# Hamedkiri/heuristique_style_transfer_code

Hardware: NVIDIA B200
Metric: images/sec (higher is better)
Workload: dtype tf32

## Files before the change

heuristique_style_transfer_code_b200/csrc/gramhead.cu:

```cuda
#include "../../include/gramhead.h"
#include "common.cuh"
#include "gram_fwd.cuh"
#include "gram_fwd_pair.cuh"
#include "gram_bwd.cuh"
#include "gram_bwd2.cuh"
#include "gram_bwd_pair.cuh"
#include "attn_head.cuh"
#include "umma_gemm.cuh"
#include "tgemm_pair.cuh"
#include "attn_head2.cuh"
#include "preprocess.cuh"
#include "transpose.cuh"
#include "patchgan.cuh"
#include "pool.cuh"
#include "stem.cuh"
#include "style_loss.cuh"
#include <string>

namespace gh {

static int sm_count_cached() {
  static int cached[64] = {0};
  int dev = 0;
  if (cudaGetDevice(&dev) != cudaSuccess || dev < 0 || dev >= 64) return 148;
// ... 309 lines not shown
          e3 = cudaFuncSetAttribute(gram_bwd_pair_kernel<KIND, MODE, NHWC, ATS, CH>,                                   \
                                    cudaFuncAttributeMaxDynamicSharedMemorySize, (int)kBpSmemBytes);                   \
          if (e3 != cudaSuccess) return (int)e3;                                                                       \
          gram_bwd_pair_kernel<KIND, MODE, NHWC, ATS, CH><<<2 * npairs, kBpThreads, kBpSmemBytes, st>>>(q, tmF, tmD);  \
        }
#define GH_LAUNCH_BP2(KIND, MODE, ATS, CH)                                                                             \
        {                                                                                                              \
          if (nhwc) GH_LAUNCH_BP(KIND, MODE, true, ATS, CH) else GH_LAUNCH_BP(KIND, MODE, false, ATS, CH)              \
        }
#define GH_LAUNCH_BP3(KIND)                                                                                            \
        {                                                                                                              \
          if (mode != GRAM_POOL) GH_LAUNCH_BP2(KIND, GRAM_DENSE, false, 1)                                             \
          else if (!ats) GH_LAUNCH_BP2(KIND, GRAM_POOL, false, 1)                                                      \
          else if (ch == 2) GH_LAUNCH_BP2(KIND, GRAM_POOL, true, 2)                                                    \
          else GH_LAUNCH_BP2(KIND, GRAM_POOL, true, 1)                                                                 \
        }
        if (is_bf16) GH_LAUNCH_BP3(KIND_BF16) else GH_LAUNCH_BP3(KIND_TF32)
#undef GH_LAUNCH_BP3
#undef GH_LAUNCH_BP2
#undef GH_LAUNCH_BP
        return (int)cudaGetLastError();
      }
    }
  }
  if (nhwc || df16) return GH_ERR_UNSUPPORTED;
  if (g_opt_bwd_variant == 2) {
    GramBwd2Params q;
    q.F = F; q.img_stride = img_stride; q.row_stride = row_stride;
    q.B = B; q.C = C; q.HW = HW; q.mode = mode;
    q.dP = dP; q.dp_img_stride = dp_img_stride; q.g = g; q.kshift = p.kshift; q.dG = dG;
    q.dF = dF; q.df_img_stride = df_img_stride; q.df_row_stride = df_row_stride; q.scale = p.scale;
    const int nhw = g_opt_bwd_nhw ? g_opt_bwd_nhw : 256;
    q.nHT = (HW + nhw - 1) / nhw;
    q.nCP = (C + 255) / 256;
    q.nkb = (C + 63) / 64;
    q.nA = (C > 128) ? 2 : 1;
    const long long total2 = (long long)B * q.nHT * q.nCP;
    if (total2 > 0x7fffffffLL) return GH_ERR_UNSUPPORTED;
    q.total_units = (int)total2;
    const int sms2 = sm_count_cached();
    const int ctas2 = (max_ctas > 0 && max_ctas < sms2) ? max_ctas : sms2;
    int grid2 = (int)(total2 < ctas2 ? total2 : ctas2);
    q.units_per_cta = (int)((total2 + grid2 - 1) / grid2);
    grid2 = (int)((total2 + q.units_per_cta - 1) / q.units_per_cta);
    q.df_vec_ok = (HW % 4 == 0 && df_img_stride % 4 == 0 && df_row_stride % 4 == 0 && ((uintptr_t)dF) % 16 == 0) ? 1 : 0;
    const bool s4 = (HW % 4 == 0) && (row_stride % 4 == 0) && (img_stride % 4 == 0);
    int src;
    if (f_dtype == GH_DTYPE_F32) src = (s4 && ((uintptr_t)F) % 16 == 0) ? 0 : 1;
    else src = (s4 && ((uintptr_t)F) % 8 == 0) ? 2 : 3;
    cudaError_t e2 = cudaErrorInvalidValue;
#define GH_LAUNCH_B2(SRC, NHW, NPW)                                                                                    \
    {                                                                                                                  \
      e2 = cudaFuncSetAttribute(gram_bwd2_kernel<SRC, NHW, NPW>, cudaFuncAttributeMaxDynamicSharedMemorySize,          \
                                (int)kB2SmemBytes);                                                                    \
      if (e2 == cudaSuccess) {                                                                                         \
        gram_bwd2_kernel<SRC, NHW, NPW><<<grid2, (NPW == 8 ? 13 : 20) * 32, kB2SmemBytes, st>>>(q);                    \
        e2 = cudaGetLastError();                                                                                       \
      }                                                                                                                \
    }
    if (nhw == 128) {
      if (src == 0) GH_LAUNCH_B2(0, 128, 8) else if (src == 1) GH_LAUNCH_B2(1, 128, 8)
      else if (src == 2) GH_LAUNCH_B2(2, 128, 8) else GH_LAUNCH_B2(3, 128, 8)
    } else if (g_opt_bwd_producer_warps == 8) {
      if (src == 0) GH_LAUNCH_B2(0, 256, 8) else if (src == 1) GH_LAUNCH_B2(1, 256, 8)
      else if (src == 2) GH_LAUNCH_B2(2, 256, 8) else GH_LAUNCH_B2(3, 256, 8)
    } else {
      if (src == 0) GH_LAUNCH_B2(0, 256, 16) else if (src == 1) GH_LAUNCH_B2(1, 256, 16)
      else if (src == 2) GH_LAUNCH_B2(2, 256, 16) else GH_LAUNCH_B2(3, 256, 16)
    }
#undef GH_LAUNCH_B2
    return (int)e2;
  }
  p.dF = dF; p.df_img_stride = df_img_stride; p.df_row_stride = df_row_stride;
  p.NB = (C > 256) ? 2 : 1;
  p.nHT = (HW + 127) / 128;
  p.nCB = (C + 256 * p.NB - 1) / (256 * p.NB);
  p.nkb = (C + 63) / 64;
  p.stage_bytes = kGbATileBytes + (uint32_t)p.NB * kGbBBlkBytes;
  p.stages = (int)(kGbRingBytes / p.stage_bytes);
  if (p.stages > kGbMaxStages) p.stages = kGbMaxStages;
  p.nacc = (p.NB == 1) ? 2 : 1;
  const long long total = (long long)B * p.nHT * p.nCB;
  if (total > 0x7fffffffLL) return GH_ERR_UNSUPPORTED;
  p.total_units = (int)total;
  const int sms = sm_count_cached();
  const int ctas = (max_ctas > 0 && max_ctas < sms) ? max_ctas : sms;
  const int grid = (int)(total < ctas ? total : ctas);
  cudaError_t e;
  if (f_dtype == GH_DTYPE_F32) {
    e = cudaFuncSetAttribute(gram_bwd_kernel<0>, cudaFuncAttributeMaxDynamicSharedMemorySize, (int)kGbSmemBytes);
    if (e != cudaSuccess) return (int)e;
    gram_bwd_kernel<0><<<grid, kGbThreads, kGbSmemBytes, st>>>(p);
  } else {
    e = cudaFuncSetAttribute(gram_bwd_kernel<2>, cudaFuncAttributeMaxDynamicSharedMemorySize, (int)kGbSmemBytes);
    if (e != cudaSuccess) return (int)e;
    gram_bwd_kernel<2><<<grid, kGbThreads, kGbSmemBytes, st>>>(p);
  }
  return (int)cudaGetLastError();
}

__device__ __forceinline__ int bin_start(int i, int C, int g) { return (int)(((long long)i * C) / g); }
__device__ __forceinline__ int bin_end(int i, int C, int g) { return (int)((((long long)(i + 1)) * C + g - 1) / g); }

__global__ void adaptive_pool_fwd_kernel(const float* __restrict__ G, int C, int g, float* __restrict__ desc,
                                         long long desc_img_stride) {
  const int i = blockIdx.x, b = blockIdx.y;
  const int r0 = bin_start(i, C, g), r1 = bin_end(i, C, g);
  const float* Gb = G + (long long)b * C * C;
  const int warp = threadIdx.x >> 5, lane = threadIdx.x & 31;
  for (int j = warp; j < g; j += 8) {
    const int c0 = bin_start(j, C, g), c1 = bin_end(j, C, g);
    const int w = c1 - c0, n = (r1 - r0) * w;
    float s = 0.f;
    for (int t = lane; t < n; t += 32) s += Gb[(long long)(r0 + t / w) * C + c0 + t % w];
#pragma unroll
    for (int o = 16; o > 0; o >>= 1) s += __shfl_xor_sync(0xffffffffu, s, o);
    if (lane == 0) desc[(long long)b * desc_img_stride + i * g + j] = s / (float)n;
  }
}
__global__ void adaptive_pool_bwd_kernel(const float* __restrict__ d_desc, long long desc_img_stride, int C, int g,
                                         float* __restrict__ dG) {
  const long long idx = (long long)blockIdx.x * blockDim.x + threadIdx.x;
  if (idx >= (long long)C * C) return;
  const int b = blockIdx.y;
  const int c = (int)(idx / C), d = (int)(idx % C);
  const float* dp = d_desc + (long long)b * desc_img_stride;
  int ilo = (int)(((long long)c * g) / C);
  while (ilo > 0 && bin_end(ilo - 1, C, g) > c) --ilo;
  int jlo = (int)(((long long)d * g) / C);
  while (jlo > 0 && bin_end(jlo - 1, C, g) > d) --jlo;
  float s = 0.f;
  for (int i = ilo; i < g && bin_start(i, C, g) <= c; ++i) {
    if (bin_end(i, C, g) <= c) continue;
    const float ni = (float)(bin_end(i, C, g) - bin_start(i, C, g));
    for (int j = jlo; j < g && bin_start(j, C, g) <= d; ++j) {
      if (bin_end(j, C, g) <= d) continue;
      const float nj = (float)(bin_end(j, C, g) - bin_start(j, C, g));
      s += dp[i * g + j] / (ni * nj);
    }
  }
  dG[(long long)b * C * C + idx] = s;
}

template <typename T>
static int stem_conv_pool_launch(StemConvPoolParams<T>& p, long long img_stride, long long c_stride, long long y_stride,
                                 long long x_stride, int B, int H, int W, void* stream) {
  p.s_img = img_stride; p.s_c = c_stride; p.s_y = y_stride; p.s_x = x_stride;
  p.B = B; p.OH = H / 2; p.OW = W / 2;
  p.PH = (p.OH - 1) / 2 + 1;
  p.PW = (p.OW - 1) / 2 + 1;
  p.tiles = (p.PW + kScTileCols - 1) / kScTileCols;
  p.vec2 = x_stride == 1 && (uintptr_t)p.x % (2 * sizeof(T)) == 0 && (img_stride % 2 == 0) && (c_stride % 2 == 0) &&
           (y_stride % 2 == 0);
  p.units = (long long)B * p.tiles * p.PH;
  const int sms = sm_count_cached();
  const int grid = (int)(p.units < sms ? p.units : sms);
  const uint32_t smem = sizeof(T) == 1 ? kScSmemBytesU8 : kScSmemBytes;
  cudaError_t e = cudaFuncSetAttribute(stem_conv_pool_kernel<T>, cudaFuncAttributeMaxDynamicSharedMemorySize, (int)smem);
  if (e != cudaSuccess) return (int)e;
  stem_conv_pool_kernel<T><<<grid, kScThreads, smem, (cudaStream_t)stream>>>(p);
  return (int)cudaGetLastError();
}

}

using namespace gh;

extern "C" {

int gh_version(void) { return 100; }

int gh_sm_count(void) { return sm_count_cached(); }

#ifdef GH_BP_PROFILE
int gh_bp_profile_read(unsigned long long* out) {
  unsigned long long zero[16] = {0};
  cudaError_t e = cudaDeviceSynchronize();
  if (e == cudaSuccess) e = cudaMemcpyFromSymbol(out, g_bp_prof, sizeof(zero));
  if (e == cudaSuccess) e = cudaMemcpyToSymbol(g_bp_prof, zero, sizeof(zero));
  return (int)e;
}
#endif

int gh_gram_bwd_plan(int C, int HW, int g, int f_dtype, int channels_last, int* out) {
  if (!out || C <= 0 || HW <= 0 || g <= 0 || (f_dtype != GH_DTYPE_F32 && f_dtype != GH_DTYPE_BF16)) return GH_ERR_BAD_ARG;
  if (C % g != 0 || g > kBpMaxG || C / g < 8 || ilog2_exact(C / g) < 0) return GH_ERR_UNSUPPORTED;
  GramBwdPairParams q;
  bool ats = false;
  int ch = 1;
  if (!plan_bwd_pair(C, HW, g, GRAM_POOL, f_dtype == GH_DTYPE_BF16, channels_last != 0, q, &ats, &ch)) return GH_ERR_UNSUPPORTED;
  out[0] = q.NT; out[1] = q.nHT; out[2] = ats ? 1 : 0; out[3] = ch; out[4] = q.a_stages; out[5] = q.b_stages;
  out[6] = q.a_tmem_base + q.a_stages * q.a_tmem_cols;
  out[7] = q.b_stages * q.b_stage_bytes + q.a_smem_tiles * (int)kBpTileBytes;
  return 0;
}

int gh_set_option(const char* name, int value) {
  if (!name) return GH_ERR_BAD_ARG;
  const std::string key(name);
  if (key == "gram_fwd_producer_warps") {
    if (value != 0 && value != 8 && value != 16) return GH_ERR_BAD_ARG;
    g_opt_fwd_producer_warps = value;
    return 0;
  }
  if (key == "gram_fwd_pair") {
    if (value < -1 || value > 1) return GH_ERR_BAD_ARG;
    g_opt_fwd_pair = value;
    return 0;
  }
  if (key == "gram_bwd_pair") {
    if (value < -1 || value > 1) return GH_ERR_BAD_ARG;
    g_opt_bwd_pair = value;
    return 0;
  }
  if (key == "gram_bwd_nt") {
    if (value != 0 && (value < 64 || value > 256 || value % 16)) return GH_ERR_BAD_ARG;
    g_opt_bwd_nt = value;
    return 0;
  }
  if (key == "gram_bwd_stages") {
    const int a = value >> 4, b = value & 15;
    if (value != 0 && (a < kBpGroups || b < 2 || a > kBpRingTiles - 2 || b > kBpMaxStages)) return GH_ERR_BAD_ARG;
    g_opt_bwd_stages = value;
    return 0;
  }
  if (key == "gram_bwd_ats") {
    if (value < -1 || value > 1) return GH_ERR_BAD_ARG;
    g_opt_bwd_ats = value;
    return 0;
  }
  if (key == "gram_bwd_ch") {
    if (value < 0 || value > 2) return GH_ERR_BAD_ARG;
    g_opt_bwd_ch = value;
    return 0;
  }
  if (key == "tma_f32_type") {
    if (value != 0 && value != 1) return GH_ERR_BAD_ARG;
    g_opt_tma_f32_type = value;
    return 0;
  }
  if (key == "gram_fwd_epilogue_warps") {
    if (value != 0 && value != 4 && value != 8) return GH_ERR_BAD_ARG;
    g_opt_fwd_epilogue_warps = value;
    return 0;
  }
  if (key == "tgemm_tn") {
    if (value != 0 && value != 128 && value != 256) return GH_ERR_BAD_ARG;
    g_opt_tg_tn = value;
    return 0;
  }
  if (key == "pdl") {
    if (value != 0 && value != 1) return GH_ERR_BAD_ARG;
    g_opt_pdl = value;
    return 0;
  }
  if (key == "attn_gemm") {
    if (value != 0 && value != 1) return GH_ERR_BAD_ARG;
    g_opt_attn_gemm = value;
    return 0;
  }
  if (key == "gram_bwd_variant") {
    if (value != 1 && value != 2) return GH_ERR_BAD_ARG;
    g_opt_bwd_variant = value;
    return 0;
  }
  if (key == "gram_bwd_producer_warps") {
    if (value != 8 && value != 16) return GH_ERR_BAD_ARG;
    g_opt_bwd_producer_warps = value;
    return 0;
  }
  if (key == "gram_bwd_nhw") {
    if (value != 0 && value != 128 && value != 256) return GH_ERR_BAD_ARG;
    g_opt_bwd_nhw = value;
    return 0;
  }
  return GH_ERR_BAD_ARG;
}

int gh_last_device_error(unsigned int* out4) {
  if (!out4) return GH_ERR_BAD_ARG;
  volatile unsigned int* rec = error_record_host();
  if (!rec) return GH_ERR_UNSUPPORTED;
  for (int i = 0; i < 4; ++i) out4[i] = rec[i];
  for (int i = 3; i >= 0; --i) rec[i] = 0u;
  return 0;
}

int gh_gram_pool_fwd(const void* F, int f_dtype, long long img_stride, long long row_stride, long long x_stride, int B,
                     int C, int HW, int g, float* desc, int l, int L, int ksplit, int max_ctas, void* stream) {
  if (!desc || l < 0 || l >= L || g <= 0) return GH_ERR_BAD_ARG;
  return gram_fwd_common(F, f_dtype, img_stride, row_stride, x_stride, B, C, HW, GRAM_POOL, g, desc + (long long)l * g * g,
                         (long long)L * g * g, ksplit, max_ctas, (cudaStream_t)stream);
}

int gh_gram_dense_fwd(const void* F, int f_dtype, long long img_stride, long long row_stride, long long x_stride, int B,
                      int C, int HW, float* G, int ksplit, int max_ctas, void* stream) {
  return gram_fwd_common(F, f_dtype, img_stride, row_stride, x_stride, B, C, HW, GRAM_DENSE, 0, G, (long long)C * C, ksplit,
                         max_ctas, (cudaStream_t)stream);
}

int gh_adaptive_pool_fwd(const float* G, int B, int C, int g, float* desc, int l, int L, void* stream) {
  if (!G || !desc || B <= 0 || C <= 0 || g <= 0 || l < 0 || l >= L) return GH_ERR_BAD_ARG;
  if (B > 65535) return GH_ERR_UNSUPPORTED;
  adaptive_pool_fwd_kernel<<<dim3(g, B), 256, 0, (cudaStream_t)stream>>>(G, C, g, desc + (long long)l * g * g,
                                                                         (long long)L * g * g);
  return (int)cudaGetLastError();
}

int gh_adaptive_pool_bwd(const float* d_desc, int l, int L, int B, int C, int g, float* dG, void* stream) {
  if (!dG || !d_desc || B <= 0 || C <= 0 || g <= 0 || l < 0 || l >= L) return GH_ERR_BAD_ARG;
  if (B > 65535) return GH_ERR_UNSUPPORTED;
  const long long n = (long long)C * C;
  adaptive_pool_bwd_kernel<<<dim3((unsigned)((n + 255) / 256), B), 256, 0, (cudaStream_t)stream>>>(
      d_desc + (long long)l * g * g, (long long)L * g * g, C, g, dG);
  return (int)cudaGetLastError();
}

int gh_gram_pool_bwd(const void* F, int f_dtype, long long img_stride, long long row_stride, long long x_stride, int B,
                     int C, int HW, int g, const float* d_desc, int l, int L, void* dF, int df_dtype,
                     long long df_img_stride, long long df_row_stride, long long df_x_stride, int max_ctas, void* stream) {
  if (!d_desc || l < 0 || l >= L || g <= 0) return GH_ERR_BAD_ARG;
  return gram_bwd_common(F, f_dtype, img_stride, row_stride, x_stride, B, C, HW, GRAM_POOL, g,
                         d_desc + (long long)l * g * g, (long long)L * g * g, nullptr, dF, df_dtype, df_img_stride,
                         df_row_stride, df_x_stride, max_ctas, (cudaStream_t)stream);
}

int gh_gram_dense_bwd(const void* F, int f_dtype, long long img_stride, long long row_stride, long long x_stride, int B,
                      int C, int HW, const float* dG, void* dF, int df_dtype, long long df_img_stride,
                      long long df_row_stride, long long df_x_stride, int max_ctas, void* stream) {
  return gram_bwd_common(F, f_dtype, img_stride, row_stride, x_stride, B, C, HW, GRAM_DENSE, 0, nullptr, 0, dG, dF,
                         df_dtype, df_img_stride, df_row_stride, df_x_stride, max_ctas, (cudaStream_t)stream);
}
// ... 443 lines not shown
```

heuristique_style_transfer_code_b200/csrc/stem.cuh:

```cuda
#pragma once
#include "common.cuh"
#include "preprocess.cuh"

namespace gh {

constexpr int kScProducerWarps = 8;
constexpr int kScEpiWarp0 = 8;
constexpr int kScMmaWarp = 12;
constexpr int kScThreads = 13 * 32;
constexpr int kScTileCols = 63;
constexpr int kScCells = 131;
constexpr int kScItems = 3 * kScCells;
constexpr int kScItemIters = (kScItems + 31) / 32;
constexpr int kScSlots = 12;
constexpr int kScAccSlots = 8;
constexpr uint32_t kScSlotBytes = kScCells * 16;
constexpr uint32_t kScPlaneBytes = kScSlots * kScSlotBytes;
constexpr uint32_t kScWBytes = 16 * 2 * 2048;
constexpr uint32_t kScAOff = kScWBytes;
constexpr uint32_t kScBiasOff = kScAOff + 4 * kScPlaneBytes;
constexpr uint32_t kScXbufOff = kScBiasOff + 64 * 4;
constexpr uint32_t kScBarOff = kScXbufOff + 2 * 4 * 64 * 4;
constexpr uint32_t kScBarBytes = 8 * (2 * kScSlots + 2 * kScAccSlots) + 16;
constexpr uint32_t kScSmemBytes = kScBarOff + kScBarBytes + 1024;
constexpr uint32_t kScTableOff = kScBarOff + kScBarBytes;
constexpr uint32_t kScSmemBytesU8 = kScSmemBytes + 3 * 256 * 4;

template <typename T>
struct StemConvPoolParams {
  const T* x;
  long long s_img, s_c, s_y, s_x;
  const float* w;
  const float* bias;
  float* out;
  int B, OH, OW, PH, PW, tiles;
  int vec2;
  long long units;
  float mean[3], std[3];
};

__device__ __forceinline__ float max_nan(float a, float b) { return (b > a || b != b) ? b : a; }

struct ScSeg {
  int b, j, py0, py1, y_lo, y_hi;
};
template <typename T>
__device__ __forceinline__ bool sc_next(const StemConvPoolParams<T>& p, long long& u, long long u1, ScSeg& s) {
  if (u >= u1) return false;
  const long long bj = u / p.PH;
  const long long end = (bj + 1) * p.PH < u1 ? (bj + 1) * p.PH : u1;
  s.b = (int)(bj / p.tiles);
  s.j = (int)(bj - (long long)s.b * p.tiles);
  s.py0 = (int)(u - bj * p.PH);
  s.py1 = s.py0 + (int)(end - u);
  s.y_lo = 2 * s.py0 - 1 > 0 ? 2 * s.py0 - 1 : 0;
  s.y_hi = 2 * s.py1 - 1 < p.OH - 1 ? 2 * s.py1 - 1 : p.OH - 1;
  u = end;
  return true;
}

__device__ __forceinline__ float4 sc_load_block(const StemConvPoolParams<float>& p, const float* q, const float*) {
  if (p.vec2) {
    const float2 t0 = __ldg(reinterpret_cast<const float2*>(q));
    const float2 t1 = __ldg(reinterpret_cast<const float2*>(q + p.s_y));
    return make_float4(t0.x, t0.y, t1.x, t1.y);
  }
  return make_float4(__ldg(q), __ldg(q + p.s_x), __ldg(q + p.s_y), __ldg(q + p.s_y + p.s_x));
}

__device__ __forceinline__ float4 sc_load_block(const StemConvPoolParams<uint8_t>& p, const uint8_t* q,
                                                const float* table) {
  uint32_t b0, b1, b2, b3;
  if (p.vec2) {
    const uint32_t t0 = __ldg(reinterpret_cast<const unsigned short*>(q));
    const uint32_t t1 = __ldg(reinterpret_cast<const unsigned short*>(q + p.s_y));
    b0 = t0 & 0xffu; b1 = t0 >> 8; b2 = t1 & 0xffu; b3 = t1 >> 8;
  } else {
    b0 = __ldg(q); b1 = __ldg(q + p.s_x); b2 = __ldg(q + p.s_y); b3 = __ldg(q + p.s_y + p.s_x);
  }
  return make_float4(table[b0], table[b1], table[b2], table[b3]);
}

template <typename T>
__global__ void __launch_bounds__(kScThreads, 1) stem_conv_pool_kernel(const StemConvPoolParams<T> p) {
  extern __shared__ uint8_t smem_raw[];
  const uint32_t raw = smem_u32(smem_raw);
  const uint32_t base = (raw + 1023u) & ~1023u;
  uint8_t* gbase = smem_raw + (base - raw);
  const uint32_t w_smem = base, a_smem = base + kScAOff;
  const float* bias_s = reinterpret_cast<const float*>(gbase + kScBiasOff);
  float* xbuf = reinterpret_cast<float*>(gbase + kScXbufOff);
  const uint32_t bar_full = base + kScBarOff, bar_empty = bar_full + 8 * kScSlots;
  const uint32_t bar_afull = bar_empty + 8 * kScSlots, bar_aempty = bar_afull + 8 * kScAccSlots;
  const uint32_t tmem_slot = bar_aempty + 8 * kScAccSlots;
  volatile uint32_t* tmem_slot_ptr = reinterpret_cast<volatile uint32_t*>(gbase + (tmem_slot - base));
  const int warp = threadIdx.x >> 5, lane = threadIdx.x & 31;

  {
    const float4* wg = reinterpret_cast<const float4*>(p.w);
    float4* ws = reinterpret_cast<float4*>(gbase);
    for (int i = threadIdx.x; i < (int)(kScWBytes / 16); i += kScThreads) ws[i] = __ldg(wg + i);
    if (threadIdx.x < 64) reinterpret_cast<float*>(gbase + kScBiasOff)[threadIdx.x] = __ldg(p.bias + threadIdx.x);
    float4* z = reinterpret_cast<float4*>(gbase + kScAOff + 3 * kScPlaneBytes);
    for (int i = threadIdx.x; i < (int)(kScPlaneBytes / 16); i += kScThreads) z[i] = make_float4(0.f, 0.f, 0.f, 0.f);
    if constexpr (sizeof(T) == 1) {
      float* table = reinterpret_cast<float*>(gbase + kScTableOff);
      for (int i = threadIdx.x; i < 3 * 256; i += kScThreads) {
        const int c = i >> 8;
        table[i] = to_tensor_normalize((unsigned)(i & 255), c == 0 ? p.mean[0] : c == 1 ? p.mean[1] : p.mean[2],
                                       c == 0 ? p.std[0] : c == 1 ? p.std[1] : p.std[2]);
      }
    }
    fence_proxy_async_smem();
  }
  if (threadIdx.x == 0) {
    for (int s = 0; s < kScSlots; ++s) {
      mbar_init(bar_full + 8 * s, 1);
      mbar_init(bar_empty + 8 * s, 1);
    }
    for (int s = 0; s < kScAccSlots; ++s) {
      mbar_init(bar_afull + 8 * s, 1);
      mbar_init(bar_aempty + 8 * s, 4);
    }
    mbar_fence_init();
  }
  if (warp == kScMmaWarp) tmem_alloc(tmem_slot, 512);
  tc_fence_before_sync();
  __syncthreads();
  tc_fence_after_sync();
  const uint32_t tmem_base = *tmem_slot_ptr;

  const long long u0 = p.units * blockIdx.x / gridDim.x, u1 = p.units * (blockIdx.x + 1) / gridDim.x;

  if (warp < kScProducerWarps) {
    uint32_t gs = 0;
    long long u = u0;
    ScSeg sg;
    while (sc_next(p, u, u1, sg)) {
      const int n_stage = sg.y_hi - sg.y_lo + 4;
      const T* img = p.x + (long long)sg.b * p.s_img;
      for (int k = 0; k < n_stage; ++k) {
        const uint32_t g = gs + (uint32_t)k;
        if ((int)(g % kScProducerWarps) != warp) continue;
        const uint32_t slot = g % kScSlots;
        const int Y = sg.y_lo + k - 2;
        const bool row_ok = Y >= 0 && Y < p.OH;
        float4 v[kScItemIters];
#pragma unroll
        for (int it = 0; it < kScItemIters; ++it) {
          const int i = it * 32 + lane;
          const int c = i / kScCells, s = i - c * kScCells;
          const int X = kScTileCols * 2 * sg.j + s - 3;
          v[it] = make_float4(0.f, 0.f, 0.f, 0.f);
          if (i < kScItems && row_ok && X >= 0 && X < p.OW) {
            const T* q = img + (long long)c * p.s_c + (long long)(2 * Y) * p.s_y + (long long)(2 * X) * p.s_x;
            v[it] = sc_load_block(p, q, reinterpret_cast<const float*>(gbase + kScTableOff) + c * 256);
          }
        }
        mbar_wait(bar_empty + 8 * slot, ((g / kScSlots) & 1u) ^ 1u, 300u + slot);
#pragma unroll
        for (int it = 0; it < kScItemIters; ++it) {
          const int i = it * 32 + lane;
          if (i < kScItems) {
            const int c = i / kScCells, s = i - c * kScCells;
            sts_u4(a_smem + (uint32_t)c * kScPlaneBytes + slot * kScSlotBytes + (uint32_t)s * 16u, tf32_rna(v[it].x),
                   tf32_rna(v[it].y), tf32_rna(v[it].z), tf32_rna(v[it].w));
          }
        }
        fence_proxy_async_smem();
        __syncwarp();
        if (lane == 0) mbar_arrive(bar_full + 8 * slot);
      }
      gs += (uint32_t)n_stage;
    }
  } else if (warp == kScMmaWarp) {
    constexpr uint32_t idesc = make_idesc_tf32(128, 64);
    const uint64_t adesc0 = make_smem_desc_noswz(a_smem, kScPlaneBytes, 128);
    const uint64_t bdesc0 = make_smem_desc_noswz(w_smem, 1024, 128);
    uint32_t gs = 0, gc = 0;
    long long u = u0;
    ScSeg sg;
    while (sc_next(p, u, u1, sg)) {
      const int n_conv = sg.y_hi - sg.y_lo + 1;
      for (int k = 0; k < n_conv; ++k, ++gc) {
        const uint32_t acc = gc % kScAccSlots;
        mbar_wait(bar_aempty + 8 * acc, ((gc / kScAccSlots) & 1u) ^ 1u, 400u + acc);
        uint32_t slot[4];
#pragma unroll
        for (int a = 0; a < 4; ++a) {
          const uint32_t g = gs + (uint32_t)(k + a);
          slot[a] = g % kScSlots;
          mbar_wait(bar_full + 8 * slot[a], (g / kScSlots) & 1u, 500u + slot[a]);
        }
        tc_fence_after_sync();
        if (elect_one()) {
          const uint32_t d = tmem_base + acc * 64u;
#pragma unroll
          for (int a = 0; a < 4; ++a) {
            const uint64_t arow = adesc0 + ((slot[a] * kScSlotBytes) >> 4);
#pragma unroll
            for (int b = 0; b < 4; ++b)
#pragma unroll
              for (int h = 0; h < 2; ++h) {
                const uint64_t da = arow + ((b * 16 + h * 2 * kScPlaneBytes) >> 4);
                const uint64_t db = bdesc0 + ((((a * 4 + b) * 2 + h) * 2048) >> 4);
                umma_tf32(d, da, db, idesc, (a | b | h) != 0);
              }
          }
          umma_commit(bar_afull + 8 * acc);
          umma_commit(bar_empty + 8 * slot[0]);
          if (k == n_conv - 1)
            for (int a = 1; a < 4; ++a) umma_commit(bar_empty + 8 * slot[a]);
        }
        __syncwarp();
      }
      gs += (uint32_t)(n_conv + 3);
    }
  } else {
    const int quad = warp - kScEpiWarp0;
    const uint32_t tlane = tmem_base + ((uint32_t)(32 * quad) << 16);
    const float neg_inf = -__int_as_float(0x7f800000);
    uint32_t gc = 0, xb = 0;
    long long u = u0;
    ScSeg sg;
    while (sc_next(p, u, u1, sg)) {
      const int x = kScTileCols * 2 * sg.j - 1 + 32 * quad + lane;
      const bool col_ok = x >= 0 && x < p.OW;
      auto acc_of = [&](int y) { return (gc + (uint32_t)(y - sg.y_lo)) % kScAccSlots; };
      auto wait_row = [&](int y) {
        const uint32_t g = gc + (uint32_t)(y - sg.y_lo);
        mbar_wait(bar_afull + 8 * (g % kScAccSlots), (g / kScAccSlots) & 1u, 600u + g % kScAccSlots);
      };
      for (int py = sg.py0; py < sg.py1; ++py) {
        const int ya = 2 * py - 1, yb = 2 * py, yc = 2 * py + 1;
        const bool ha = ya >= sg.y_lo, hc = yc <= sg.y_hi;
        if (py == sg.py0 && ha) wait_row(ya);
        wait_row(yb);
        if (hc) wait_row(yc);
        tc_fence_after_sync();
        float m[64];
#pragma unroll
        for (int h = 0; h < 2; ++h) {
          uint32_t r[32];
          tmem_ld32_nowait(tlane + acc_of(yb) * 64u + 32u * h, r);
          tmem_ld_wait();
#pragma unroll
          for (int i = 0; i < 32; ++i) m[32 * h + i] = __uint_as_float(r[i]);
          if (ha) {
            tmem_ld32_nowait(tlane + acc_of(ya) * 64u + 32u * h, r);
            tmem_ld_wait();
#pragma unroll
            for (int i = 0; i < 32; ++i) m[32 * h + i] = max_nan(m[32 * h + i], __uint_as_float(r[i]));
          }
          if (hc) {
            tmem_ld32_nowait(tlane + acc_of(yc) * 64u + 32u * h, r);
            tmem_ld_wait();
#pragma unroll
            for (int i = 0; i < 32; ++i) m[32 * h + i] = max_nan(m[32 * h + i], __uint_as_float(r[i]));
          }
        }
        tc_fence_before_sync();
        __syncwarp();
        if (lane == 0) {
          if (ha) mbar_arrive(bar_aempty + 8 * acc_of(ya));
          mbar_arrive(bar_aempty + 8 * acc_of(yb));
          if (hc && py == sg.py1 - 1) mbar_arrive(bar_aempty + 8 * acc_of(yc));
        }
        if (!col_ok) {
#pragma unroll
          for (int i = 0; i < 64; ++i) m[i] = neg_inf;
        }
        float* xs = xbuf + xb * 256;
        if (lane == 0 && quad > 0) {
#pragma unroll
          for (int i = 0; i < 64; i += 4)
            *reinterpret_cast<float4*>(xs + quad * 64 + i) = make_float4(m[i], m[i + 1], m[i + 2], m[i + 3]);
        }
        asm volatile("bar.sync 1, 128;" ::: "memory");
        const bool from_next = lane == 30 && quad < 3;
        const int qx = 16 * quad + (lane >> 1);
        const int px = kScTileCols * sg.j + qx;
        const bool store = !(lane & 1) && qx < kScTileCols && px < p.PW;
        float4* o = reinterpret_cast<float4*>(p.out + (((long long)sg.b * p.PH + py) * p.PW + px) * 64);
#pragma unroll
        for (int i = 0; i < 64; i += 4) {
          float r4[4];
#pragma unroll
          for (int e = 0; e < 4; ++e) {
            const float v1 = __shfl_down_sync(0xffffffffu, m[i + e], 1);
            float v2 = __shfl_down_sync(0xffffffffu, m[i + e], 2);
            if (from_next) v2 = xs[(quad + 1) * 64 + i + e];
            float t = max_nan(max_nan(m[i + e], v1), v2) + bias_s[i + e];
            r4[e] = t != t ? t : fmaxf(t, 0.f);
          }
          if (store) o[i / 4] = make_float4(r4[0], r4[1], r4[2], r4[3]);
        }
        xb ^= 1u;
      }
      gc += (uint32_t)(sg.y_hi - sg.y_lo + 1);
    }
  }

  tc_fence_before_sync();
  __syncthreads();
  if (warp == kScMmaWarp) {
    tc_fence_after_sync();
    tmem_dealloc(tmem_base, 512);
  }
}

}
```

Before: 43890.

## Rebalance stem conv-pool warps, split epilogue by channel halves, trim UMMA work

Reassigns warps in the stem conv+pool kernel: seven producer warps and eight epilogue warps, with each group of four epilogue warps handling one half of the 64 output channels and using its own named barrier. The epilogue now issues its TMEM loads back to back and carries the bottom conv row forward in registers, so each accumulator row is loaded once instead of twice. The MMA issue skips the zero third plane for odd k-steps by using separate descriptors, which removes the zero-filled plane and its shared memory. It also swaps the hand-written NaN-propagating max for the max.NaN instruction, moves unit indexing to 32-bit, and adds optional clock64 profiling. The risks are lower producer throughput with one fewer warp and correctness of the new descriptor strides.

After: 45960, median of 6. 1.05x the previous value.

```diff
diff --git a/heuristique_style_transfer_code_b200/csrc/gramhead.cu b/heuristique_style_transfer_code_b200/csrc/gramhead.cu
--- a/heuristique_style_transfer_code_b200/csrc/gramhead.cu
+++ b/heuristique_style_transfer_code_b200/csrc/gramhead.cu
@@ -485,9 +485,11 @@
   p.tiles = (p.PW + kScTileCols - 1) / kScTileCols;
   p.vec2 = x_stride == 1 && (uintptr_t)p.x % (2 * sizeof(T)) == 0 && (img_stride % 2 == 0) && (c_stride % 2 == 0) &&
            (y_stride % 2 == 0);
-  p.units = (long long)B * p.tiles * p.PH;
+  const long long units = (long long)B * p.tiles * p.PH;
+  if (units >= (1ll << 30)) return GH_ERR_UNSUPPORTED;
+  p.units = (int)units;
   const int sms = sm_count_cached();
-  const int grid = (int)(p.units < sms ? p.units : sms);
+  const int grid = p.units < sms ? p.units : sms;
   const uint32_t smem = sizeof(T) == 1 ? kScSmemBytesU8 : kScSmemBytes;
   cudaError_t e = cudaFuncSetAttribute(stem_conv_pool_kernel<T>, cudaFuncAttributeMaxDynamicSharedMemorySize, (int)smem);
   if (e != cudaSuccess) return (int)e;
@@ -511,6 +513,16 @@
   cudaError_t e = cudaDeviceSynchronize();
   if (e == cudaSuccess) e = cudaMemcpyFromSymbol(out, g_bp_prof, sizeof(zero));
   if (e == cudaSuccess) e = cudaMemcpyToSymbol(g_bp_prof, zero, sizeof(zero));
+  return (int)e;
+}
+#endif
+
+#ifdef GH_SC_PROFILE
+int gh_sc_profile_read(unsigned long long* out) {
+  unsigned long long zero[16] = {0};
+  cudaError_t e = cudaDeviceSynchronize();
+  if (e == cudaSuccess) e = cudaMemcpyFromSymbol(out, g_sc_prof, sizeof(zero));
+  if (e == cudaSuccess) e = cudaMemcpyToSymbol(g_sc_prof, zero, sizeof(zero));
   return (int)e;
 }
 #endif
diff --git a/heuristique_style_transfer_code_b200/csrc/stem.cuh b/heuristique_style_transfer_code_b200/csrc/stem.cuh
--- a/heuristique_style_transfer_code_b200/csrc/stem.cuh
+++ b/heuristique_style_transfer_code_b200/csrc/stem.cuh
@@ -4,10 +4,11 @@
 
 namespace gh {
 
-constexpr int kScProducerWarps = 8;
-constexpr int kScEpiWarp0 = 8;
-constexpr int kScMmaWarp = 12;
-constexpr int kScThreads = 13 * 32;
+constexpr int kScProducerWarps = 7;
+constexpr int kScEpiWarp0 = kScProducerWarps;
+constexpr int kScEpiWarps = 8;
+constexpr int kScMmaWarp = kScEpiWarp0 + kScEpiWarps;
+constexpr int kScThreads = (kScMmaWarp + 1) * 32;
 constexpr int kScTileCols = 63;
 constexpr int kScCells = 131;
 constexpr int kScItems = 3 * kScCells;
@@ -18,7 +19,7 @@
 constexpr uint32_t kScPlaneBytes = kScSlots * kScSlotBytes;
 constexpr uint32_t kScWBytes = 16 * 2 * 2048;
 constexpr uint32_t kScAOff = kScWBytes;
-constexpr uint32_t kScBiasOff = kScAOff + 4 * kScPlaneBytes;
+constexpr uint32_t kScBiasOff = kScAOff + 3 * kScPlaneBytes;
 constexpr uint32_t kScXbufOff = kScBiasOff + 64 * 4;
 constexpr uint32_t kScBarOff = kScXbufOff + 2 * 4 * 64 * 4;
 constexpr uint32_t kScBarBytes = 8 * (2 * kScSlots + 2 * kScAccSlots) + 16;
@@ -35,24 +36,43 @@
   float* out;
   int B, OH, OW, PH, PW, tiles;
   int vec2;
-  long long units;
+  int units;
   float mean[3], std[3];
 };
 
-__device__ __forceinline__ float max_nan(float a, float b) { return (b > a || b != b) ? b : a; }
+#ifdef GH_SC_PROFILE
+__device__ unsigned long long g_sc_prof[16];
+#define GH_SC_DECL(var) long long var = 0
+#define GH_SC_CLK(var) const long long var = clock64()
+#define GH_SC_ADD(acc, var) acc += clock64() - var
+#define GH_SC_FLUSH(slot, acc) atomicAdd(&g_sc_prof[slot], (unsigned long long)(acc))
+#define GH_SC_INC(var) ++var
+#else
+#define GH_SC_DECL(var)
+#define GH_SC_CLK(var)
+#define GH_SC_ADD(acc, var)
+#define GH_SC_FLUSH(slot, acc)
+#define GH_SC_INC(var)
+#endif
+
+__device__ __forceinline__ float max_nan(float a, float b) {
+  float r;
+  asm("max.NaN.f32 %0, %1, %2;" : "=f"(r) : "f"(a), "f"(b));
+  return r;
+}
 
 struct ScSeg {
   int b, j, py0, py1, y_lo, y_hi;
 };
 template <typename T>
-__device__ __forceinline__ bool sc_next(const StemConvPoolParams<T>& p, long long& u, long long u1, ScSeg& s) {
+__device__ __forceinline__ bool sc_next(const StemConvPoolParams<T>& p, int& u, int u1, ScSeg& s) {
   if (u >= u1) return false;
-  const long long bj = u / p.PH;
-  const long long end = (bj + 1) * p.PH < u1 ? (bj + 1) * p.PH : u1;
-  s.b = (int)(bj / p.tiles);
-  s.j = (int)(bj - (long long)s.b * p.tiles);
-  s.py0 = (int)(u - bj * p.PH);
-  s.py1 = s.py0 + (int)(end - u);
+  const int bj = u / p.PH;
+  const int end = (bj + 1) * p.PH < u1 ? (bj + 1) * p.PH : u1;
+  s.b = bj / p.tiles;
+  s.j = bj - s.b * p.tiles;
+  s.py0 = u - bj * p.PH;
+  s.py1 = s.py0 + (end - u);
   s.y_lo = 2 * s.py0 - 1 > 0 ? 2 * s.py0 - 1 : 0;
   s.y_hi = 2 * s.py1 - 1 < p.OH - 1 ? 2 * s.py1 - 1 : p.OH - 1;
   u = end;
@@ -83,6 +103,7 @@
 
 template <typename T>
 __global__ void __launch_bounds__(kScThreads, 1) stem_conv_pool_kernel(const StemConvPoolParams<T> p) {
+  GH_SC_CLK(prof_cta0);
   extern __shared__ uint8_t smem_raw[];
   const uint32_t raw = smem_u32(smem_raw);
   const uint32_t base = (raw + 1023u) & ~1023u;
@@ -101,8 +122,6 @@
     float4* ws = reinterpret_cast<float4*>(gbase);
     for (int i = threadIdx.x; i < (int)(kScWBytes / 16); i += kScThreads) ws[i] = __ldg(wg + i);
     if (threadIdx.x < 64) reinterpret_cast<float*>(gbase + kScBiasOff)[threadIdx.x] = __ldg(p.bias + threadIdx.x);
-    float4* z = reinterpret_cast<float4*>(gbase + kScAOff + 3 * kScPlaneBytes);
-    for (int i = threadIdx.x; i < (int)(kScPlaneBytes / 16); i += kScThreads) z[i] = make_float4(0.f, 0.f, 0.f, 0.f);
     if constexpr (sizeof(T) == 1) {
       float* table = reinterpret_cast<float*>(gbase + kScTableOff);
       for (int i = threadIdx.x; i < 3 * 256; i += kScThreads) {
@@ -120,7 +139,7 @@
     }
     for (int s = 0; s < kScAccSlots; ++s) {
       mbar_init(bar_afull + 8 * s, 1);
-      mbar_init(bar_aempty + 8 * s, 4);
+      mbar_init(bar_aempty + 8 * s, kScEpiWarps);
     }
     mbar_fence_init();
   }
@@ -130,12 +149,17 @@
   tc_fence_after_sync();
   const uint32_t tmem_base = *tmem_slot_ptr;
 
-  const long long u0 = p.units * blockIdx.x / gridDim.x, u1 = p.units * (blockIdx.x + 1) / gridDim.x;
+  const int u0 = (int)((long long)p.units * blockIdx.x / gridDim.x);
+  const int u1 = (int)((long long)p.units * (blockIdx.x + 1) / gridDim.x);
 
   if (warp < kScProducerWarps) {
     uint32_t gs = 0;
-    long long u = u0;
+    int u = u0;
     ScSeg sg;
+    GH_SC_DECL(prof_wait);
+    GH_SC_DECL(prof_store);
+    GH_SC_DECL(prof_n);
+    GH_SC_CLK(prof_t0);
     while (sc_next(p, u, u1, sg)) {
       const int n_stage = sg.y_hi - sg.y_lo + 4;
       const T* img = p.x + (long long)sg.b * p.s_img;
@@ -157,7 +181,11 @@
             v[it] = sc_load_block(p, q, reinterpret_cast<const float*>(gbase + kScTableOff) + c * 256);
           }
         }
+        GH_SC_CLK(prof_w0);
         mbar_wait(bar_empty + 8 * slot, ((g / kScSlots) & 1u) ^ 1u, 300u + slot);
+        GH_SC_ADD(prof_wait, prof_w0);
+        GH_SC_CLK(prof_s0);
+        GH_SC_INC(prof_n);
 #pragma unroll
         for (int it = 0; it < kScItemIters; ++it) {
           const int i = it * 32 + lane;
@@ -170,21 +198,40 @@
         fence_proxy_async_smem();
         __syncwarp();
         if (lane == 0) mbar_arrive(bar_full + 8 * slot);
+        GH_SC_ADD(prof_store, prof_s0);
       }
       gs += (uint32_t)n_stage;
     }
+#ifdef GH_SC_PROFILE
+    if (warp == 0 && lane == 0) {
+      long long prof_tot = 0;
+      GH_SC_ADD(prof_tot, prof_t0);
+      GH_SC_FLUSH(4, prof_tot);
+      GH_SC_FLUSH(5, prof_wait);
+      GH_SC_FLUSH(6, prof_store);
+      GH_SC_FLUSH(7, prof_n);
+    }
+#endif
   } else if (warp == kScMmaWarp) {
     constexpr uint32_t idesc = make_idesc_tf32(128, 64);
     const uint64_t adesc0 = make_smem_desc_noswz(a_smem, kScPlaneBytes, 128);
     const uint64_t bdesc0 = make_smem_desc_noswz(w_smem, 1024, 128);
+    const uint64_t adesc2 = make_smem_desc_noswz(a_smem + 2 * kScPlaneBytes, 16, 128);
+    const uint64_t bdesc2 = make_smem_desc_noswz(w_smem + 2048, 4096, 128);
     uint32_t gs = 0, gc = 0;
-    long long u = u0;
+    int u = u0;
     ScSeg sg;
+    GH_SC_DECL(prof_ae);
+    GH_SC_DECL(prof_full);
+    GH_SC_CLK(prof_t0);
     while (sc_next(p, u, u1, sg)) {
       const int n_conv = sg.y_hi - sg.y_lo + 1;
       for (int k = 0; k < n_conv; ++k, ++gc) {
         const uint32_t acc = gc % kScAccSlots;
+        GH_SC_CLK(prof_w0);
         mbar_wait(bar_aempty + 8 * acc, ((gc / kScAccSlots) & 1u) ^ 1u, 400u + acc);
+        GH_SC_ADD(prof_ae, prof_w0);
+        GH_SC_CLK(prof_w1);
         uint32_t slot[4];
 #pragma unroll
         for (int a = 0; a < 4; ++a) {
@@ -192,20 +239,19 @@
           slot[a] = g % kScSlots;
           mbar_wait(bar_full + 8 * slot[a], (g / kScSlots) & 1u, 500u + slot[a]);
         }
+        GH_SC_ADD(prof_full, prof_w1);
         tc_fence_after_sync();
         if (elect_one()) {
           const uint32_t d = tmem_base + acc * 64u;
 #pragma unroll
           for (int a = 0; a < 4; ++a) {
-            const uint64_t arow = adesc0 + ((slot[a] * kScSlotBytes) >> 4);
+            const uint32_t row = (slot[a] * kScSlotBytes) >> 4;
 #pragma unroll
             for (int b = 0; b < 4; ++b)
-#pragma unroll
-              for (int h = 0; h < 2; ++h) {
-                const uint64_t da = arow + ((b * 16 + h * 2 * kScPlaneBytes) >> 4);
-                const uint64_t db = bdesc0 + ((((a * 4 + b) * 2 + h) * 2048) >> 4);
-                umma_tf32(d, da, db, idesc, (a | b | h) != 0);
-              }
+              umma_tf32(d, adesc0 + row + b, bdesc0 + (((a * 4 + b) * 2 * 2048) >> 4), idesc, (a | b) != 0);
+#pragma unroll
+            for (int b = 0; b < 4; b += 2)
+              umma_tf32(d, adesc2 + row + b, bdesc2 + (((a * 4 + b) * 2 * 2048) >> 4), idesc, 1u);
           }
           umma_commit(bar_afull + 8 * acc);
           umma_commit(bar_empty + 8 * slot[0]);
@@ -216,13 +262,30 @@
       }
       gs += (uint32_t)(n_conv + 3);
     }
+#ifdef GH_SC_PROFILE
+    if (lane == 0) {
+      long long prof_tot = 0;
+      GH_SC_ADD(prof_tot, prof_t0);
+      GH_SC_FLUSH(0, prof_tot);
+      GH_SC_FLUSH(1, prof_ae);
+      GH_SC_FLUSH(2, prof_full);
+      GH_SC_FLUSH(3, gc);
+    }
+#endif
   } else {
-    const int quad = warp - kScEpiWarp0;
-    const uint32_t tlane = tmem_base + ((uint32_t)(32 * quad) << 16);
+    const int quad = warp & 3, half = (warp - kScEpiWarp0) >> 2;
+    const uint32_t tlane = tmem_base + ((uint32_t)(32 * quad) << 16) + 32u * (uint32_t)half;
+    const float* bias_h = bias_s + 32 * half;
     const float neg_inf = -__int_as_float(0x7f800000);
     uint32_t gc = 0, xb = 0;
-    long long u = u0;
+    int u = u0;
     ScSeg sg;
+    GH_SC_DECL(prof_af);
+    GH_SC_DECL(prof_ld);
+    GH_SC_DECL(prof_bar);
+    GH_SC_DECL(prof_st);
+    GH_SC_DECL(prof_n);
+    GH_SC_CLK(prof_t0);
     while (sc_next(p, u, u1, sg)) {
       const int x = kScTileCols * 2 * sg.j - 1 + 32 * quad + lane;
       const bool col_ok = x >= 0 && x < p.OW;
@@ -231,74 +294,88 @@
         const uint32_t g = gc + (uint32_t)(y - sg.y_lo);
         mbar_wait(bar_afull + 8 * (g % kScAccSlots), (g / kScAccSlots) & 1u, 600u + g % kScAccSlots);
       };
+      uint32_t ra[32];
       for (int py = sg.py0; py < sg.py1; ++py) {
         const int ya = 2 * py - 1, yb = 2 * py, yc = 2 * py + 1;
-        const bool ha = ya >= sg.y_lo, hc = yc <= sg.y_hi;
-        if (py == sg.py0 && ha) wait_row(ya);
+        const bool ha = ya >= sg.y_lo, hc = yc <= sg.y_hi, first = py == sg.py0;
+        GH_SC_CLK(prof_w0);
+        if (first && ha) wait_row(ya);
         wait_row(yb);
         if (hc) wait_row(yc);
+        GH_SC_ADD(prof_af, prof_w0);
+        GH_SC_CLK(prof_l0);
+        GH_SC_INC(prof_n);
         tc_fence_after_sync();
-        float m[64];
-#pragma unroll
-        for (int h = 0; h < 2; ++h) {
-          uint32_t r[32];
-          tmem_ld32_nowait(tlane + acc_of(yb) * 64u + 32u * h, r);
-          tmem_ld_wait();
-#pragma unroll
-          for (int i = 0; i < 32; ++i) m[32 * h + i] = __uint_as_float(r[i]);
-          if (ha) {
-            tmem_ld32_nowait(tlane + acc_of(ya) * 64u + 32u * h, r);
-            tmem_ld_wait();
-#pragma unroll
-            for (int i = 0; i < 32; ++i) m[32 * h + i] = max_nan(m[32 * h + i], __uint_as_float(r[i]));
-          }
-          if (hc) {
-            tmem_ld32_nowait(tlane + acc_of(yc) * 64u + 32u * h, r);
-            tmem_ld_wait();
-#pragma unroll
-            for (int i = 0; i < 32; ++i) m[32 * h + i] = max_nan(m[32 * h + i], __uint_as_float(r[i]));
-          }
-        }
+        uint32_t rb[32], rc[32];
+        if (first && ha) tmem_ld32_nowait(tlane + acc_of(ya) * 64u, ra);
+        tmem_ld32_nowait(tlane + acc_of(yb) * 64u, rb);
+        if (hc) tmem_ld32_nowait(tlane + acc_of(yc) * 64u, rc);
+        tmem_ld_wait();
         tc_fence_before_sync();
         __syncwarp();
         if (lane == 0) {
-          if (ha) mbar_arrive(bar_aempty + 8 * acc_of(ya));
+          if (first && ha) mbar_arrive(bar_aempty + 8 * acc_of(ya));
           mbar_arrive(bar_aempty + 8 * acc_of(yb));
-          if (hc && py == sg.py1 - 1) mbar_arrive(bar_aempty + 8 * acc_of(yc));
-        }
+          if (hc) mbar_arrive(bar_aempty + 8 * acc_of(yc));
+        }
+        float m[32];
+#pragma unroll
+        for (int i = 0; i < 32; ++i) {
+          m[i] = __uint_as_float(rb[i]);
+          if (ha) m[i] = max_nan(m[i], __uint_as_float(ra[i]));
+          if (hc) m[i] = max_nan(m[i], __uint_as_float(rc[i]));
+          ra[i] = rc[i];
+        }
+        GH_SC_ADD(prof_ld, prof_l0);
         if (!col_ok) {
 #pragma unroll
-          for (int i = 0; i < 64; ++i) m[i] = neg_inf;
-        }
-        float* xs = xbuf + xb * 256;
+          for (int i = 0; i < 32; ++i) m[i] = neg_inf;
+        }
+        float* xs = xbuf + xb * 256 + 32 * half;
         if (lane == 0 && quad > 0) {
 #pragma unroll
-          for (int i = 0; i < 64; i += 4)
+          for (int i = 0; i < 32; i += 4)
             *reinterpret_cast<float4*>(xs + quad * 64 + i) = make_float4(m[i], m[i + 1], m[i + 2], m[i + 3]);
         }
-        asm volatile("bar.sync 1, 128;" ::: "memory");
+        GH_SC_CLK(prof_b0);
+        asm volatile("bar.sync %0, 128;" ::"r"(1 + half) : "memory");
+        GH_SC_ADD(prof_bar, prof_b0);
+        GH_SC_CLK(prof_s0);
         const bool from_next = lane == 30 && quad < 3;
         const int qx = 16 * quad + (lane >> 1);
         const int px = kScTileCols * sg.j + qx;
         const bool store = !(lane & 1) && qx < kScTileCols && px < p.PW;
-        float4* o = reinterpret_cast<float4*>(p.out + (((long long)sg.b * p.PH + py) * p.PW + px) * 64);
-#pragma unroll
-        for (int i = 0; i < 64; i += 4) {
+        float4* o = reinterpret_cast<float4*>(p.out + (((long long)sg.b * p.PH + py) * p.PW + px) * 64 + 32 * half);
+#pragma unroll
+        for (int i = 0; i < 32; i += 4) {
           float r4[4];
 #pragma unroll
           for (int e = 0; e < 4; ++e) {
             const float v1 = __shfl_down_sync(0xffffffffu, m[i + e], 1);
             float v2 = __shfl_down_sync(0xffffffffu, m[i + e], 2);
             if (from_next) v2 = xs[(quad + 1) * 64 + i + e];
-            float t = max_nan(max_nan(m[i + e], v1), v2) + bias_s[i + e];
-            r4[e] = t != t ? t : fmaxf(t, 0.f);
+            float t = max_nan(max_nan(m[i + e], v1), v2) + bias_h[i + e];
+            r4[e] = max_nan(t, 0.f);
           }
           if (store) o[i / 4] = make_float4(r4[0], r4[1], r4[2], r4[3]);
         }
         xb ^= 1u;
+        GH_SC_ADD(prof_st, prof_s0);
       }
       gc += (uint32_t)(sg.y_hi - sg.y_lo + 1);
     }
+#ifdef GH_SC_PROFILE
+    if (warp == kScEpiWarp0 && lane == 0) {
+      long long prof_tot = 0;
+      GH_SC_ADD(prof_tot, prof_t0);
+      GH_SC_FLUSH(8, prof_tot);
+      GH_SC_FLUSH(9, prof_af);
+      GH_SC_FLUSH(10, prof_ld);
+      GH_SC_FLUSH(11, prof_bar);
+      GH_SC_FLUSH(12, prof_st);
+      GH_SC_FLUSH(13, prof_n);
+    }
+#endif
   }
 
   tc_fence_before_sync();
@@ -307,6 +384,14 @@
     tc_fence_after_sync();
     tmem_dealloc(tmem_base, 512);
   }
-}
-
-}
+#ifdef GH_SC_PROFILE
+  if (threadIdx.x == 0) {
+    long long prof_tot = 0;
+    GH_SC_ADD(prof_tot, prof_cta0);
+    GH_SC_FLUSH(14, 1);
+    GH_SC_FLUSH(15, prof_tot);
+  }
+#endif
+}
+
+}
```
